# jesusdpa1/ssqueeze_rs

Hardware: NVIDIA B200
Metric: ssq_stft input Msamples/s (higher is better)
Workload: dtype f32

## Files before the change

### ssqueeze_rs_b200/csrc/stft_h32r.cuh

```cuda
#pragma once
#include "fft_regs.cuh"

#ifndef H32R_PK
#define H32R_PK(MODE) true
#endif
#define H32R_AS 261

__device__ __forceinline__ int h32r_phys(int k) { return k + (k >> 6); }

struct H32RItem {
  int kb;
  float vre, vim;
};

template <int MODE, int SQZ, bool DBG = false>
__device__ __forceinline__ H32RItem h32r_item(const StftParams& P, float txs, float2* col, float2* colB, float skf,
                                              float2 A, float2 B, size_t dbg_base = 0) {
  H32RItem it;
  const unsigned sgn = __float_as_uint(skf) & 0x80000000u;
  const float2 cd = add2<MODE == 0>(A, make_float2(B.x, -B.y));
  const float c = cd.x, d0 = cd.y;
  if (MODE == 1) {
    const int k = (int)fabsf(skf);
    col[h32r_phys(k)] = make_float2(0.5f * c, __uint_as_float(__float_as_uint(0.5f * d0) ^ sgn));
    if (colB) {
      const float2 ba = add2<MODE == 0>(B, make_float2(-A.x, A.y));
      const float b0 = ba.x, a = ba.y;
      colB[h32r_phys(k)] = make_float2(0.5f * a, __uint_as_float(__float_as_uint(0.5f * b0) ^ sgn));
    }
    it.kb = -1;
    it.vre = it.vim = 0.f;
    return it;
  }
  const float2 ba = add2<MODE == 0>(B, make_float2(-A.x, A.y));
  const float b0 = ba.x, a = ba.y;
  const float den = fmaf(c, c, d0 * d0);
  const float num0 = fmaf(b0, c, -a * d0);
  const float q0 = num0 * rcp_approx(den);
  const float binf = fabsf(fmaf(-q0, P.cphase, skf));
  it.kb = min(max(__float2int_ru(binf - 0.5f), 0), 256);
  if (DBG) {
    const float ms = (txs < 0.f) != (P.tx_scale < 0.f) ? -1.f : 1.f;
    ssq_dbg_emit(P, dbg_base, (int)fabsf(skf), ms * c, ms * __uint_as_float(__float_as_uint(d0) ^ sgn), ms * a,
                 ms * __uint_as_float(__float_as_uint(b0) ^ sgn), binf, den < P.gate2, it.kb);
  }
  if (den < P.gate2) it.kb = -1;
  if (SQZ == SSQ_SQUEEZE_LEBESGUE) {
    it.vre = P.leb_val;
    it.vim = 0.f;
  } else {
    it.vre = c * txs;
    it.vim = d0 * __uint_as_float(__float_as_uint(txs) ^ sgn);
  }
  return it;
}

__device__ __noinline__ void h32r_collision(float2* col, unsigned* T, int kb, float vre, float vim, bool mine,
                                            int lane) {
  const bool on = kb >= 0;
  {
    const unsigned act = __ballot_sync(0xffffffffu, on);
    const int first = __ffs(act) - 1;
    const int kb0 = __shfl_sync(0xffffffffu, kb, first);
    if (__all_sync(0xffffffffu, !on || kb == kb0)) {
      float sr = on ? vre : 0.f, si = on ? vim : 0.f;
#pragma unroll
      for (int o = 16; o > 0; o >>= 1) {
        sr += __shfl_xor_sync(0xffffffffu, sr, o);
        si += __shfl_xor_sync(0xffffffffu, si, o);
      }
      if (lane == first) smem_rmw_add(col + h32r_phys(kb0), sr, si);
      return;
    }
  }
  if (on && !mine) T[kb] = 0xFF;
  __syncwarp();
  const bool contended = on && T[kb] == 0xFF;
  if (on && !contended) smem_rmw_add(col + h32r_phys(kb), vre, vim);
  unsigned m = __ballot_sync(0xffffffffu, contended);
  if (__popc(m) > 4) {
    while (m) {
      const int first = __ffs(m) - 1;
      const int kb0 = __shfl_sync(0xffffffffu, kb, first);
      const bool member = contended && kb == kb0;
      float sr = member ? vre : 0.f, si = member ? vim : 0.f;
#pragma unroll
      for (int o = 16; o > 0; o >>= 1) {
        sr += __shfl_xor_sync(0xffffffffu, sr, o);
        si += __shfl_xor_sync(0xffffffffu, si, o);
      }
      if (lane == first) smem_rmw_add(col + h32r_phys(kb0), sr, si);
      m &= ~__ballot_sync(0xffffffffu, member);
    }
    __syncwarp();
    return;
  }
  while (m) {
    const int src = __ffs(m) - 1;
    m &= m - 1;
    if (lane == src) smem_rmw_add(col + h32r_phys(kb), vre, vim);
    __syncwarp();
  }
}

template <int MODE, int SQZ, bool DBG = false>
__device__ __forceinline__ void h32r_frame(const StftParams& P, const H32Lane& L, float skf0, float wrapd, float txs,
                                           float2* xch, float2* col, float2* colB, float2 (&va)[8], float2 (&vb)[8],
                                           size_t dbg_base = 0) {
  const int lane = L.lane;
  const bool l0 = L.l0;
  unsigned* tagA = reinterpret_cast<unsigned*>(xch);
  unsigned* tagB = tagA + 264;
  h32_fft512<true, true, H32R_PK(MODE)>(L, xch, va, vb);
  __syncwarp();

#define H32R_PAIR(r, A, B)                                   \
  float2 A = va[r], B = vb[r];                               \
  if (l0) {                                                  \
    A = (r) < 4 ? va[r] : vb[(11 - (r)) & 7];                \
    B = (r) < 4 ? va[(8 - (r)) & 7] : vb[((r)-4) & 7];       \
  }

  H32RItem cur;
  float skf = skf0;
  {
    H32R_PAIR(0, A, B)
    cur = h32r_item<MODE, SQZ, DBG>(P, txs, col, colB, skf, A, B, dbg_base);
  }
  if (MODE == 0) {
    if (cur.kb >= 0) tagA[cur.kb] = (unsigned)lane;
    __syncwarp();
  }
#pragma unroll
  for (int r = 0; r < 8; ++r) {
    H32RItem nxt;
    nxt.kb = -1;
    nxt.vre = nxt.vim = 0.f;
    if (r < 7) {
      skf += (skf >= 192.f) ? wrapd : 64.f;
      H32R_PAIR(r + 1, A, B)
      nxt = h32r_item<MODE, SQZ, DBG>(P, txs, col, colB, skf, A, B, dbg_base);
    }
    if (MODE == 0) {
      unsigned* T = (r & 1) ? tagB : tagA;
      unsigned* Tn = (r & 1) ? tagA : tagB;
      const bool on = cur.kb >= 0;
      float2* slot = col + h32r_phys(on ? cur.kb : 0);
      float2 t = *slot;
      const bool mine = !on || T[cur.kb] == (unsigned)lane;
      if (__all_sync(0xffffffffu, mine)) {
        if (on) {
          t.x += cur.vre;
          t.y += cur.vim;
          *slot = t;
        }
      } else {
        h32r_collision(col, T, cur.kb, cur.vre, cur.vim, mine, lane);
      }
      if (r < 7 && nxt.kb >= 0) Tn[nxt.kb] = (unsigned)lane;
      __syncwarp();
    }
    cur = nxt;
  }
#undef H32R_PAIR
  if (l0) {
    const H32RItem it = h32r_item<MODE, SQZ, DBG>(P, txs, col, colB, 256.f, va[4], va[4], dbg_base);
    if (MODE == 0 && it.kb >= 0) smem_rmw_add(col + h32r_phys(it.kb), it.vre, it.vim);
  }
  __syncwarp();
}

__device__ __noinline__ float h32r_edge_sample(const float* x, int64_t n, int64_t p, int left, int padtype,
                                               int64_t origin) {
  return stft_sample<false>(x, n, p, left, padtype, origin);
}

#define H32R_NW(MODE) ((MODE) == 1 ? 8 : 4)

template <int MODE, int SQZ, bool SLIDE, bool DBG = false>
__global__ void __launch_bounds__(H32R_NW(MODE) * 32, 16 / H32R_NW(MODE)) ssq_stft512_h32r_kernel(const StftParams P) {
  constexpr int N = 512, AS = H32R_AS, NW = H32R_NW(MODE), F = 4 * NW;
  constexpr bool PAIR = (MODE == 1) && SLIDE;
  extern __shared__ float2 smem[];
  float2* wtab = smem;
  float2* tw2tab = smem + N;
  float2* acc = smem + N + 72;
  const int lane = threadIdx.x & 31, warp = threadIdx.x >> 5;
  float2* xch = acc + F * AS + warp * N;

  for (int i = threadIdx.x; i < N; i += blockDim.x) wtab[i] = make_float2(P.win[i], P.dwin[i]);
  if (threadIdx.x < 64)
    tw2tab[(threadIdx.x >> 3) * 9 + (threadIdx.x & 7)] = P.tw[((threadIdx.x >> 3) * (threadIdx.x & 7) * 8) & (N - 1)];
  for (int i = threadIdx.x; i < F * AS; i += blockDim.x) acc[i] = make_float2(0.f, 0.f);

  H32Lane L;
  L.lane = lane;
  L.j2 = lane ? 64 - lane : 32;
  L.tw2 = tw2tab + (lane & 7) * 9;
  const int rho = lane & 7;
  const int ea = lane + 64 * rho;
#pragma unroll
  for (int t = 1; t < 8; ++t) {
    L.tw3a[t - 1] = P.tw[(ea * t) & (N - 1)];
    L.tw3b[t - 1] = make_float2(0.f, 0.f);
  }
  L.f1 = (lane >> 1) & 3;
  L.rd1a = (lane >> 3) * 8 + ((((lane & 7) >> 1) ^ ((lane >> 4) & 3)) << 1) + (lane & 1);
  L.rd1b = ((lane >> 3) + 4) * 8 + ((((lane & 7) >> 1) ^ (((lane >> 4) + 2) & 3)) << 1) + (lane & 1);
  L.g2 = (lane >> 3) & 1;
  L.wr2 = (lane >> 3) * 64 + (lane & 7);
  L.lane_f = (float)lane;
  L.j2_f = (float)L.j2;
  L.l0 = (lane == 0);
  const float txs = (P.modulated && (lane & 1)) ? -P.tx_scale : P.tx_scale;
  float skf0, wrapd;
  if (lane == 0) {
    skf0 = 0.f;
    wrapd = -160.f;
  } else {
    const int ka = lane + 64 * rho;
    skf0 = rho <= 3 ? (float)ka : (float)(ka - 512);
    wrapd = -448.f;
  }
  __syncthreads();

  const float* xc = nullptr;
  int64_t f0 = 0;
  int nfr = 0;
  bool inner = false;
  float xw[17];
  const int64_t lo = P.left + P.x_origin;
  const int tpc = (int)P.tiles_per_channel, ntiles = (int)P.total_tiles;
  auto open_tile = [&](int tile) {
    const int ch = tile / tpc;
    f0 = (int64_t)(tile - ch * tpc) * F + 4 * warp;
    nfr = (int)max((int64_t)0, min((int64_t)4, P.n_frames - f0));
    f0 += P.frame0;
    xc = P.x + (size_t)ch * P.x_stride;
    const int64_t hop = SLIDE ? 32 : P.hop;
    inner = f0 * hop - P.left >= 0 && (f0 + 3) * hop + N - 1 - P.left + (PAIR ? 32 : 0) < P.n;
    if (nfr > 0) {
      const int64_t p = f0 * hop + lane;
      if (inner) {
#pragma unroll
        for (int j = 0; j < (PAIR ? 17 : 16); ++j) xw[j] = __ldg(xc + (p + 32 * j - lo));
      } else {
#pragma unroll
        for (int j = 0; j < (PAIR ? 17 : 16); ++j) xw[j] = h32r_edge_sample(xc, P.n, p + 32 * j, P.left, P.padtype, P.x_origin);
      }
    }
  };

  for (int tile = (int)blockIdx.x - (int)gridDim.x; tile < ntiles; tile += (int)gridDim.x) {
    const bool real = tile >= 0;
    const int tch = real ? tile / tpc : 0;
    const int64_t tf0 = real ? (int64_t)(tile - tch * tpc) * F : 0;
    const int tnf = real ? (int)min((int64_t)F, P.n_frames - tf0) : 0;
    const int next = tile + (int)gridDim.x;
    const int my_n = real ? nfr : 0;
#pragma unroll 1
    for (int s = 0; s < 4; s += (PAIR ? 2 : 1)) {
      const bool active = s < my_n;
      float2 va[8], vb[8];
      if (active) {
#pragma unroll
        for (int t = 0; t < 8; ++t) {
          const float2 w0 = wtab[lane + 64 * t], w1 = wtab[lane + 32 + 64 * t];
          if (PAIR) {
            va[t] = mul2<false>(make_float2(xw[2 * t], xw[2 * t + 1]), bc2(w0.x));
            vb[t] = mul2<false>(make_float2(xw[2 * t + 1], xw[2 * t + 2]), bc2(w1.x));
          } else {
            va[t] = mul2(bc2(xw[2 * t]), w0);
            vb[t] = mul2(bc2(xw[2 * t + 1]), w1);
          }
        }
      }
      if (s == (PAIR ? 2 : 3)) {
        if (next < ntiles) open_tile(next);
      } else if (s + (PAIR ? 2 : 1) < my_n) {
        if (PAIR) {
#pragma unroll
          for (int j = 0; j < 15; ++j) xw[j] = xw[j + 2];
          const int64_t p = (f0 + s + 2) * 32 + lane + 480;
          if (inner) {
            xw[15] = __ldg(xc + (p - lo));
            xw[16] = __ldg(xc + (p + 32 - lo));
          } else {
            xw[15] = h32r_edge_sample(xc, P.n, p, P.left, P.padtype, P.x_origin);
            xw[16] = h32r_edge_sample(xc, P.n, p + 32, P.left, P.padtype, P.x_origin);
          }
        } else if (SLIDE) {
#pragma unroll
          for (int j = 0; j < 15; ++j) xw[j] = xw[j + 1];
          const int64_t p = (f0 + s + 1) * 32 + lane + 480;
          xw[15] = inner ? __ldg(xc + (p - lo)) : h32r_edge_sample(xc, P.n, p, P.left, P.padtype, P.x_origin);
        } else {
          const int64_t p = (f0 + s + 1) * (int64_t)P.hop + lane;
          if (inner) {
#pragma unroll
            for (int j = 0; j < 16; ++j) xw[j] = __ldg(xc + (p + 32 * j - lo));
          } else {
#pragma unroll
            for (int j = 0; j < 16; ++j) xw[j] = h32r_edge_sample(xc, P.n, p + 32 * j, P.left, P.padtype, P.x_origin);
          }
        }
      }
      if (active)
        h32r_frame<MODE, SQZ, DBG>(P, L, skf0, wrapd, txs, xch, acc + (4 * warp + s) * AS,
                                   PAIR ? acc + (4 * warp + s + 1) * AS : nullptr, va, vb,
                                   DBG ? (size_t)tch * 257 * P.n_frames + tf0 + 4 * warp + s : 0);
    }
    if (!real) continue;
    __syncthreads();
    {
      const int fr = threadIdx.x % F, v = threadIdx.x / F;
      float2* a = acc + fr * AS + v;
      float2* g = P.out + ((size_t)tch * 257 + v) * P.n_frames + tf0 + fr;
      const size_t gstep = (size_t)8 * P.n_frames;
      const bool ok = fr < tnf;
#pragma unroll 1
      for (int io = 0; io < 4; ++io) {
#pragma unroll
        for (int ii = 0; ii < 8; ++ii) {
          const float2 val = a[8 * ii];
          if (MODE == 0) a[8 * ii] = make_float2(0.f, 0.f);
          if (ok) __stcs(g, val);
          g += gstep;
        }
        a += 65;
      }
      if (v == 0) {
        const float2 val = a[0];
        if (MODE == 0) a[0] = make_float2(0.f, 0.f);
        if (ok) __stcs(g, val);
      }
    }
    __syncthreads();
  }
}

static ssq_status stft_h32r_launch(ssq_ctx* ctx, StftParams& P, bool* done) {
  *done = false;
  if (P.n_fft != 512 || ctx->opt.no_h32r) return SSQ_OK;
  const int NW = H32R_NW(P.mode), F = 4 * NW;
  P.F = F;
  P.acc_stride = H32R_AS;
  P.tiles_per_channel = (P.n_frames + F - 1) / F;
  P.total_tiles = P.tiles_per_channel * P.channels;
  if (P.total_tiles > (int64_t)0x7ff00000) return SSQ_OK;
  *done = true;
  const size_t smem = ((size_t)512 + 72 + (size_t)F * H32R_AS + (size_t)NW * 512) * sizeof(float2);
  const int grid = (int)std::min<int64_t>(P.total_tiles, (int64_t)ctx->num_sms * (16 / NW));
  const bool leb = P.squeezing == SSQ_SQUEEZE_LEBESGUE;
  void (*k)(const StftParams);
  const bool dbg = P.mode == 0 && (P.aux_Sx || P.aux_dSx || P.aux_w || P.aux_kb);
  if (dbg)
    k = P.hop == 32 ? (leb ? ssq_stft512_h32r_kernel<0, 1, true, true> : ssq_stft512_h32r_kernel<0, 0, true, true>)
                    : (leb ? ssq_stft512_h32r_kernel<0, 1, false, true> : ssq_stft512_h32r_kernel<0, 0, false, true>);
  else if (P.hop == 32)
    k = P.mode == 1 ? ssq_stft512_h32r_kernel<1, 0, true>
        : leb       ? ssq_stft512_h32r_kernel<0, 1, true>
                    : ssq_stft512_h32r_kernel<0, 0, true>;
  else
    k = P.mode == 1 ? ssq_stft512_h32r_kernel<1, 0, false>
        : leb       ? ssq_stft512_h32r_kernel<0, 1, false>
                    : ssq_stft512_h32r_kernel<0, 0, false>;
  SSQ_CUDA_TRY(ctx, cudaFuncSetAttribute(k, cudaFuncAttributeMaxDynamicSharedMemorySize, (int)smem));
  k<<<grid, NW * 32, smem, ctx->stream>>>(P);
  const char* name = P.mode == 1 ? "ssq_stft512_h32r_kernel<stft>" : "ssq_stft512_h32r_kernel<ssq>";
  SSQ_TRY(ssq_check_launch(ctx, name));
  ctx->last_kernel = name;
  return SSQ_OK;
}
```

Before: 21630.

## Stage window taps and sliding input ring in tensor memory for SSQ mode

For the squeezing mode, the window and derivative-window taps move out of shared memory into Blackwell tensor memory (TMEM), allocated per CTA through tcgen05.alloc. With hop 32, the sliding input window is also kept as a TMEM ring: each step loads a shifted 16-column window and stores one new sample, instead of shifting 16 registers. This shrinks the dynamic shared memory footprint and is meant to cut register pressure and shared-memory bank traffic. In exchange it adds synchronous tcgen05 ld/st waits on every frame and alloc/dealloc plus fence overhead, and it defers prefetch of the next tile until after the frame loop, which reduces load overlap.

New measurement: 22550 (median of 6 runs). 4.3% higher.

```diff
diff --git a/ssqueeze_rs_b200/csrc/stft_h32r.cuh b/ssqueeze_rs_b200/csrc/stft_h32r.cuh
--- a/ssqueeze_rs_b200/csrc/stft_h32r.cuh
+++ b/ssqueeze_rs_b200/csrc/stft_h32r.cuh
@@ -177,18 +177,81 @@
 
 #define H32R_NW(MODE) ((MODE) == 1 ? 8 : 4)
 
+
+__device__ __forceinline__ void h32r_tmem_st32(uint32_t taddr, const float (&v)[32]) {
+  asm volatile(
+      "tcgen05.st.sync.aligned.32x32b.x32.b32 [%0], {%1,%2,%3,%4,%5,%6,%7,%8,%9,%10,%11,%12,%13,%14,%15,%16,%17,%18,%19,"
+      "%20,%21,%22,%23,%24,%25,%26,%27,%28,%29,%30,%31,%32};\n\t"
+      "tcgen05.wait::st.sync.aligned;" ::"r"(taddr),
+      "f"(v[0]), "f"(v[1]), "f"(v[2]), "f"(v[3]), "f"(v[4]), "f"(v[5]), "f"(v[6]), "f"(v[7]), "f"(v[8]), "f"(v[9]),
+      "f"(v[10]), "f"(v[11]), "f"(v[12]), "f"(v[13]), "f"(v[14]), "f"(v[15]), "f"(v[16]), "f"(v[17]), "f"(v[18]),
+      "f"(v[19]), "f"(v[20]), "f"(v[21]), "f"(v[22]), "f"(v[23]), "f"(v[24]), "f"(v[25]), "f"(v[26]), "f"(v[27]),
+      "f"(v[28]), "f"(v[29]), "f"(v[30]), "f"(v[31]));
+}
+
+__device__ __forceinline__ void h32r_tmem_st16(uint32_t taddr, const float (&v)[17]) {
+  asm volatile(
+      "tcgen05.st.sync.aligned.32x32b.x16.b32 [%0], {%1,%2,%3,%4,%5,%6,%7,%8,%9,%10,%11,%12,%13,%14,%15,%16};" ::"r"(taddr),
+      "f"(v[0]), "f"(v[1]), "f"(v[2]), "f"(v[3]), "f"(v[4]), "f"(v[5]), "f"(v[6]), "f"(v[7]), "f"(v[8]), "f"(v[9]),
+      "f"(v[10]), "f"(v[11]), "f"(v[12]), "f"(v[13]), "f"(v[14]), "f"(v[15]));
+}
+
+__device__ __forceinline__ void h32r_tmem_st1(uint32_t taddr, float v) {
+  asm volatile("tcgen05.st.sync.aligned.32x32b.x1.b32 [%0], {%1};" ::"r"(taddr), "f"(v));
+}
+
+__device__ __forceinline__ void h32r_tmem_ld_window(uint32_t taddr_x, uint32_t taddr_w, float (&x)[16], float (&v)[32]) {
+  asm volatile(
+      "tcgen05.wait::st.sync.aligned;\n\t"
+      "tcgen05.ld.sync.aligned.32x32b.x16.b32 {%0,%1,%2,%3,%4,%5,%6,%7,%8,%9,%10,%11,%12,%13,%14,%15}, [%48];\n\t"
+      "tcgen05.ld.sync.aligned.32x32b.x32.b32 {%16,%17,%18,%19,%20,%21,%22,%23,%24,%25,%26,%27,%28,%29,%30,%31,%32,%33,"
+      "%34,%35,%36,%37,%38,%39,%40,%41,%42,%43,%44,%45,%46,%47}, [%49];\n\t"
+      "tcgen05.wait::ld.sync.aligned;"
+      : "=f"(x[0]), "=f"(x[1]), "=f"(x[2]), "=f"(x[3]), "=f"(x[4]), "=f"(x[5]), "=f"(x[6]), "=f"(x[7]), "=f"(x[8]),
+        "=f"(x[9]), "=f"(x[10]), "=f"(x[11]), "=f"(x[12]), "=f"(x[13]), "=f"(x[14]), "=f"(x[15]),
+        "=f"(v[0]), "=f"(v[1]), "=f"(v[2]), "=f"(v[3]), "=f"(v[4]), "=f"(v[5]), "=f"(v[6]), "=f"(v[7]), "=f"(v[8]),
+        "=f"(v[9]), "=f"(v[10]), "=f"(v[11]), "=f"(v[12]), "=f"(v[13]), "=f"(v[14]), "=f"(v[15]), "=f"(v[16]),
+        "=f"(v[17]), "=f"(v[18]), "=f"(v[19]), "=f"(v[20]), "=f"(v[21]), "=f"(v[22]), "=f"(v[23]), "=f"(v[24]),
+        "=f"(v[25]), "=f"(v[26]), "=f"(v[27]), "=f"(v[28]), "=f"(v[29]), "=f"(v[30]), "=f"(v[31])
+      : "r"(taddr_x), "r"(taddr_w));
+}
+
+__device__ __forceinline__ void h32r_tmem_ld32(uint32_t taddr, float (&v)[32]) {
+  asm volatile(
+      "tcgen05.ld.sync.aligned.32x32b.x32.b32 {%0,%1,%2,%3,%4,%5,%6,%7,%8,%9,%10,%11,%12,%13,%14,%15,%16,%17,%18,%19,"
+      "%20,%21,%22,%23,%24,%25,%26,%27,%28,%29,%30,%31}, [%32];\n\t"
+      "tcgen05.wait::ld.sync.aligned;"
+      : "=f"(v[0]), "=f"(v[1]), "=f"(v[2]), "=f"(v[3]), "=f"(v[4]), "=f"(v[5]), "=f"(v[6]), "=f"(v[7]), "=f"(v[8]),
+        "=f"(v[9]), "=f"(v[10]), "=f"(v[11]), "=f"(v[12]), "=f"(v[13]), "=f"(v[14]), "=f"(v[15]), "=f"(v[16]),
+        "=f"(v[17]), "=f"(v[18]), "=f"(v[19]), "=f"(v[20]), "=f"(v[21]), "=f"(v[22]), "=f"(v[23]), "=f"(v[24]),
+        "=f"(v[25]), "=f"(v[26]), "=f"(v[27]), "=f"(v[28]), "=f"(v[29]), "=f"(v[30]), "=f"(v[31])
+      : "r"(taddr));
+}
+
 template <int MODE, int SQZ, bool SLIDE, bool DBG = false>
 __global__ void __launch_bounds__(H32R_NW(MODE) * 32, 16 / H32R_NW(MODE)) ssq_stft512_h32r_kernel(const StftParams P) {
   constexpr int N = 512, AS = H32R_AS, NW = H32R_NW(MODE), F = 4 * NW;
   constexpr bool PAIR = (MODE == 1) && SLIDE;
+  constexpr bool TM = MODE == 0;
+  constexpr bool RING = TM && SLIDE;
+  constexpr int TMC = RING ? 64 : 32;
+  constexpr int WT = TM ? 0 : N;
   extern __shared__ float2 smem[];
+  __shared__ uint32_t tmem_base_s;
   float2* wtab = smem;
-  float2* tw2tab = smem + N;
-  float2* acc = smem + N + 72;
+  float2* tw2tab = smem + WT;
+  float2* acc = smem + WT + 72;
   const int lane = threadIdx.x & 31, warp = threadIdx.x >> 5;
   float2* xch = acc + F * AS + warp * N;
 
-  for (int i = threadIdx.x; i < N; i += blockDim.x) wtab[i] = make_float2(P.win[i], P.dwin[i]);
+  if (TM && warp == 0) {
+    asm volatile("tcgen05.alloc.cta_group::1.sync.aligned.shared::cta.b32 [%0], %1;" ::"r"(
+                     (uint32_t)__cvta_generic_to_shared(&tmem_base_s)),
+                 "n"(TMC));
+    asm volatile("tcgen05.relinquish_alloc_permit.cta_group::1.sync.aligned;");
+  }
+  if (!TM)
+    for (int i = threadIdx.x; i < N; i += blockDim.x) wtab[i] = make_float2(P.win[i], P.dwin[i]);
   if (threadIdx.x < 64)
     tw2tab[(threadIdx.x >> 3) * 9 + (threadIdx.x & 7)] = P.tw[((threadIdx.x >> 3) * (threadIdx.x & 7) * 8) & (N - 1)];
   for (int i = threadIdx.x; i < F * AS; i += blockDim.x) acc[i] = make_float2(0.f, 0.f);
@@ -222,7 +285,22 @@
     skf0 = rho <= 3 ? (float)ka : (float)(ka - 512);
     wrapd = -448.f;
   }
+  if (TM) asm volatile("tcgen05.fence::before_thread_sync;");
   __syncthreads();
+  uint32_t taps = 0;
+  if (TM) {
+    asm volatile("tcgen05.fence::after_thread_sync;");
+    taps = tmem_base_s + ((uint32_t)(warp * 32) << 16);
+    float v[32];
+#pragma unroll
+    for (int t = 0; t < 8; ++t) {
+      v[4 * t] = P.win[lane + 64 * t];
+      v[4 * t + 1] = P.dwin[lane + 64 * t];
+      v[4 * t + 2] = P.win[lane + 32 + 64 * t];
+      v[4 * t + 3] = P.dwin[lane + 32 + 64 * t];
+    }
+    h32r_tmem_st32(taps, v);
+  }
 
   const float* xc = nullptr;
   int64_t f0 = 0;
@@ -258,17 +336,35 @@
     const int tnf = real ? (int)min((int64_t)F, P.n_frames - tf0) : 0;
     const int next = tile + (int)gridDim.x;
     const int my_n = real ? nfr : 0;
+    if (RING && real) h32r_tmem_st16(taps + 32, xw);
 #pragma unroll 1
     for (int s = 0; s < 4; s += (PAIR ? 2 : 1)) {
       const bool active = s < my_n;
       float2 va[8], vb[8];
+      float xn = 0.f;
       if (active) {
+        float tv[TM ? 32 : 1];
+        float xs[RING ? 16 : 1];
+        if constexpr (RING)
+          h32r_tmem_ld_window(taps + 32 + s, taps, xs, tv);
+        else if constexpr (TM)
+          h32r_tmem_ld32(taps, tv);
 #pragma unroll
         for (int t = 0; t < 8; ++t) {
-          const float2 w0 = wtab[lane + 64 * t], w1 = wtab[lane + 32 + 64 * t];
+          float2 w0, w1;
+          if constexpr (TM) {
+            w0 = make_float2(tv[4 * t], tv[4 * t + 1]);
+            w1 = make_float2(tv[4 * t + 2], tv[4 * t + 3]);
+          } else {
+            w0 = wtab[lane + 64 * t];
+            w1 = wtab[lane + 32 + 64 * t];
+          }
           if (PAIR) {
             va[t] = mul2<false>(make_float2(xw[2 * t], xw[2 * t + 1]), bc2(w0.x));
             vb[t] = mul2<false>(make_float2(xw[2 * t + 1], xw[2 * t + 2]), bc2(w1.x));
+          } else if constexpr (RING) {
+            va[t] = mul2(bc2(xs[2 * t]), w0);
+            vb[t] = mul2(bc2(xs[2 * t + 1]), w1);
           } else {
             va[t] = mul2(bc2(xw[2 * t]), w0);
             vb[t] = mul2(bc2(xw[2 * t + 1]), w1);
@@ -276,7 +372,7 @@
         }
       }
       if (s == (PAIR ? 2 : 3)) {
-        if (next < ntiles) open_tile(next);
+        if (!RING && next < ntiles) open_tile(next);
       } else if (s + (PAIR ? 2 : 1) < my_n) {
         if (PAIR) {
 #pragma unroll
@@ -289,6 +385,9 @@
             xw[15] = h32r_edge_sample(xc, P.n, p, P.left, P.padtype, P.x_origin);
             xw[16] = h32r_edge_sample(xc, P.n, p + 32, P.left, P.padtype, P.x_origin);
           }
+        } else if (RING) {
+          const int64_t p = (f0 + s + 1) * 32 + lane + 480;
+          xn = inner ? __ldg(xc + (p - lo)) : h32r_edge_sample(xc, P.n, p, P.left, P.padtype, P.x_origin);
         } else if (SLIDE) {
 #pragma unroll
           for (int j = 0; j < 15; ++j) xw[j] = xw[j + 1];
@@ -309,7 +408,9 @@
         h32r_frame<MODE, SQZ, DBG>(P, L, skf0, wrapd, txs, xch, acc + (4 * warp + s) * AS,
                                    PAIR ? acc + (4 * warp + s + 1) * AS : nullptr, va, vb,
                                    DBG ? (size_t)tch * 257 * P.n_frames + tf0 + 4 * warp + s : 0);
-    }
+      if (RING && s + 1 < my_n) h32r_tmem_st1(taps + 48 + s, xn);
+    }
+    if (RING && next < ntiles) open_tile(next);
     if (!real) continue;
     __syncthreads();
     {
@@ -337,6 +438,13 @@
     }
     __syncthreads();
   }
+  if (TM) {
+    asm volatile("tcgen05.fence::before_thread_sync;");
+    __syncthreads();
+    asm volatile("tcgen05.fence::after_thread_sync;");
+    if (warp == 0)
+      asm volatile("tcgen05.dealloc.cta_group::1.sync.aligned.b32 %0, %1;" ::"r"(tmem_base_s), "n"(TMC));
+  }
 }
 
 static ssq_status stft_h32r_launch(ssq_ctx* ctx, StftParams& P, bool* done) {
@@ -349,7 +457,8 @@
   P.total_tiles = P.tiles_per_channel * P.channels;
   if (P.total_tiles > (int64_t)0x7ff00000) return SSQ_OK;
   *done = true;
-  const size_t smem = ((size_t)512 + 72 + (size_t)F * H32R_AS + (size_t)NW * 512) * sizeof(float2);
+  const size_t wt = P.mode == 1 ? 512 : 0;
+  const size_t smem = (wt + 72 + (size_t)F * H32R_AS + (size_t)NW * 512) * sizeof(float2);
   const int grid = (int)std::min<int64_t>(P.total_tiles, (int64_t)ctx->num_sms * (16 / NW));
   const bool leb = P.squeezing == SSQ_SQUEEZE_LEBESGUE;
   void (*k)(const StftParams);
```
